# igashov/DiffLinker

Measured on AMD Instinct MI355X. Metric: molecules/sec (500-step sample_chain), higher is better.
Workload: dtype f32 (f16x3 split MFMA, fp32 accumulate)

## Files before the change

difflinker_amd/_lib.py:

```python
import ctypes
import os

import torch

_HERE = os.path.dirname(os.path.abspath(__file__))
LIB_PATH = os.environ.get('DIFFLINKER_HIP_LIB') or os.path.join(_HERE, 'libdifflinker_hip.so')
TEST_HOOKS_LIB_PATH = os.path.join(_HERE, 'libdifflinker_hip_testhooks.so')

DL_OK = 0
ABI_VERSION = 7
PRECISIONS = {'fp32': 0, 'f16x3': 1, 'f16x2': 2}
DL_ERR_TOO_MANY_ATOMS = -3


class DLConfig(ctypes.Structure):
    _fields_ = [
        ('n_dims', ctypes.c_int32), ('in_node_nf', ctypes.c_int32), ('context_node_nf', ctypes.c_int32),
        ('hidden_nf', ctypes.c_int32), ('n_layers', ctypes.c_int32), ('inv_sublayers', ctypes.c_int32),
        ('condition_time', ctypes.c_int32), ('norm_constant', ctypes.c_float),
        ('normalization_factor', ctypes.c_float), ('precision', ctypes.c_int32),
        ('attention', ctypes.c_int32), ('tanh', ctypes.c_int32), ('coords_range', ctypes.c_float),
        ('aggregation_mean', ctypes.c_int32), ('sin_embedding', ctypes.c_int32),
    ]

# ... 2 lines not shown
    _fields_ = [('in_node_nf', ctypes.c_int32), ('hidden_nf', ctypes.c_int32), ('out_node_nf', ctypes.c_int32),
                ('n_layers', ctypes.c_int32)]


class DLInpaintCoef(ctypes.Structure):
    _fields_ = [('alpha_ts', ctypes.c_float), ('c_eps', ctypes.c_float), ('sigma', ctypes.c_float),
                ('a_q', ctypes.c_float), ('b_q', ctypes.c_float), ('decode', ctypes.c_int32),
                ('inv_alpha0', ctypes.c_float), ('sigma0', ctypes.c_float), ('sigma_x', ctypes.c_float),
                ('norm_x', ctypes.c_float), ('norm_h', ctypes.c_float), ('bias_h', ctypes.c_float)]


class DLStepCoef(ctypes.Structure):
    _fields_ = [('t', ctypes.c_float), ('alpha_ts', ctypes.c_float), ('c_eps', ctypes.c_float),
                ('sigma', ctypes.c_float)]


class DLChainArgs(ctypes.Structure):
    _fields_ = [
        ('B', ctypes.c_int32), ('N', ctypes.c_int32), ('T', ctypes.c_int32), ('keep_frames', ctypes.c_int32),
        ('x', ctypes.c_void_p), ('h', ctypes.c_void_p), ('node_mask', ctypes.c_void_p),
        ('fragment_mask', ctypes.c_void_p), ('linker_mask', ctypes.c_void_p), ('edge_mask', ctypes.c_void_p),
        ('context', ctypes.c_void_p), ('noise_x', ctypes.c_void_p), ('noise_h', ctypes.c_void_p),
        ('noise_seed', ctypes.c_uint64), ('mol_offset', ctypes.c_int32), ('team', ctypes.c_int32),
        ('coefs', ctypes.c_void_p),
        ('inv_alpha0', ctypes.c_float), ('sigma0', ctypes.c_float), ('sigma_x', ctypes.c_float),
        ('norm_x', ctypes.c_float), ('norm_h', ctypes.c_float), ('bias_h', ctypes.c_float),
        ('chain', ctypes.c_void_p), ('nan_flags', ctypes.c_void_p), ('nan_step', ctypes.c_void_p),
        ('order', ctypes.c_void_p), ('workspace', ctypes.c_void_p), ('workspace_bytes', ctypes.c_size_t),
        ('mol_index', ctypes.c_void_p), ('order_first', ctypes.c_int32), ('order_count', ctypes.c_int32),
        ('q_begin', ctypes.c_void_p), ('q_end', ctypes.c_void_p), ('z_state', ctypes.c_void_p), ('skip_flags', ctypes.c_void_p),
    ]


LOSS_ROW = 8


class DLLossArgs(ctypes.Structure):
    _fields_ = [
        ('B', ctypes.c_int32), ('N', ctypes.c_int32), ('nf', ctypes.c_int32), ('T', ctypes.c_int32),
        ('timesteps', ctypes.c_int32), ('inpainting', ctypes.c_int32),
        ('xh', ctypes.c_void_p), ('node_mask', ctypes.c_void_p), ('fragment_mask', ctypes.c_void_p),
        ('linker_mask', ctypes.c_void_p), ('gamma_table', ctypes.c_void_p), ('noise_x', ctypes.c_void_p),
        ('noise_h', ctypes.c_void_p), ('noise_seed', ctypes.c_uint64), ('mol_offset', ctypes.c_int32),
        ('t_given', ctypes.c_int32), ('t_int', ctypes.c_void_p), ('t', ctypes.c_void_p), ('gamma', ctypes.c_void_p),
        ('z_t', ctypes.c_void_p), ('eps_hat', ctypes.c_void_p), ('norm_h', ctypes.c_float), ('bias_h', ctypes.c_float),
        ('prior', ctypes.c_void_p), ('rows', ctypes.c_void_p),
    ]


class DLBackwardArgs(ctypes.Structure):
    _fields_ = [
        ('B', ctypes.c_int32), ('N', ctypes.c_int32), ('in_node_nf', ctypes.c_int32), ('context_node_nf', ctypes.c_int32),
        ('condition_time', ctypes.c_int32), ('hidden_nf', ctypes.c_int32), ('n_layers', ctypes.c_int32),
        ('inv_sublayers', ctypes.c_int32), ('centering', ctypes.c_int32), ('norm_constant', ctypes.c_float),
        ('normalization_factor', ctypes.c_float), ('params', ctypes.c_void_p), ('n_params', ctypes.c_int64),
        ('xh', ctypes.c_void_p), ('t', ctypes.c_void_p), ('t_is_scalar', ctypes.c_int32), ('node_mask', ctypes.c_void_p),
        ('linker_mask', ctypes.c_void_p), ('edge_mask', ctypes.c_void_p), ('context', ctypes.c_void_p),
        ('grad_out', ctypes.c_void_p), ('grad_params', ctypes.c_void_p), ('workspace', ctypes.c_void_p),
        ('workspace_bytes', ctypes.c_size_t),
    ]


class DLSizeTrainArgs(ctypes.Structure):
    _fields_ = [
        ('B', ctypes.c_int32), ('N', ctypes.c_int32), ('in_node_nf', ctypes.c_int32), ('hidden_nf', ctypes.c_int32),
        ('out_node_nf', ctypes.c_int32), ('n_layers', ctypes.c_int32), ('batch_norm', ctypes.c_int32),
        ('params', ctypes.c_void_p), ('n_params', ctypes.c_int64), ('one_hot', ctypes.c_void_p),
        ('positions', ctypes.c_void_p), ('fragment_mask', ctypes.c_void_p), ('edge_mask', ctypes.c_void_p),
        ('logits', ctypes.c_void_p), ('batch_stats', ctypes.c_void_p), ('flags', ctypes.c_void_p),
        ('grad_logits', ctypes.c_void_p), ('grad_params', ctypes.c_void_p), ('workspace', ctypes.c_void_p),
        ('workspace_bytes', ctypes.c_size_t),
    ]


EXPORTS = ('dl_abi_version', 'dl_last_hip_error', 'dl_max_atoms', 'dl_error_string', 'dl_model_num_tensors',
           'dl_model_create', 'dl_model_destroy', 'dl_egnn_forward_fc', 'dl_sampler_step', 'dl_sample_chain_fc',
           'dl_set_profile_buffer', 'dl_profile_max_events', 'dl_pocket_workspace_bytes', 'dl_egnn_forward_pocket',
           'dl_size_model_num_tensors', 'dl_size_model_create', 'dl_size_model_destroy', 'dl_size_max_fragment_atoms',
           'dl_size_gnn_forward', 'dl_philox_fill', 'dl_egnn_forward_fc_large', 'dl_inpaint_step', 'dl_workspace_bytes',
           'dl_team_max', 'dl_egnn_forward_fc_team', 'dl_team_max_atoms',
           'dl_edm_loss_prologue', 'dl_edm_loss_epilogue', 'dl_edm_loss_grad', 'dl_egnn_backward_fc_num_params',
           'dl_egnn_backward_fc_workspace_bytes', 'dl_egnn_backward_max_atoms', 'dl_egnn_backward_fc',
           'dl_size_train_num_params', 'dl_size_train_workspace_bytes', 'dl_size_train_forward', 'dl_size_train_backward')
TEST_HOOK_EXPORTS = ('dl_debug_team_fault',)

_lib = None


class HipLibraryError(RuntimeError):
    pass


def load():
    global _lib
    if _lib is None:
        _lib = _open(LIB_PATH)
    return _lib


class test_hooks:

    def __enter__(self):
        global _lib
        self.saved = _lib
        lib = _open(TEST_HOOKS_LIB_PATH)
        lib.dl_debug_team_fault.restype = None
        lib.dl_debug_team_fault.argtypes = [ctypes.c_int32]
        _lib = lib
        return lib

    def __exit__(self, *exc):
        global _lib
        _lib.dl_debug_team_fault(0)
        _lib = self.saved
        return False

# ... 12 lines not shown
    lib.dl_last_hip_error.restype = i32
    lib.dl_max_atoms.restype = i32
    lib.dl_error_string.restype = ctypes.c_char_p
    lib.dl_error_string.argtypes = [i32]
    lib.dl_model_num_tensors.restype = i32
    lib.dl_model_num_tensors.argtypes = [ctypes.POINTER(DLConfig)]
    lib.dl_model_create.restype = i32
    lib.dl_model_create.argtypes = [ctypes.POINTER(DLConfig), ctypes.POINTER(vp), i32, ctypes.POINTER(vp)]
    lib.dl_model_destroy.restype = None
    lib.dl_model_destroy.argtypes = [vp]
    lib.dl_egnn_forward_fc.restype = i32
    lib.dl_egnn_forward_fc.argtypes = [vp, i32, i32, vp, vp, i32, vp, vp, vp, vp, vp, vp, vp, ctypes.c_size_t, vp]
    lib.dl_egnn_forward_fc_team.restype = i32
    lib.dl_egnn_forward_fc_team.argtypes = [vp, i32, i32, vp, vp, i32, vp, vp, vp, vp, vp, vp, i32, vp, ctypes.c_size_t, vp]
    lib.dl_workspace_bytes.restype = ctypes.c_size_t
    lib.dl_workspace_bytes.argtypes = [i32, i32]
    lib.dl_team_max.restype = i32
    lib.dl_team_max.argtypes = [i32]
    lib.dl_team_max_atoms.restype = i32
    lib.dl_team_max_atoms.argtypes = [i32]
    lib.dl_sampler_step.restype = i32
    lib.dl_sampler_step.argtypes = [i32, i32, i32, vp, vp, vp, vp, vp, DLStepCoef, vp, vp]
    lib.dl_set_profile_buffer.restype = None
    lib.dl_set_profile_buffer.argtypes = [vp]
    lib.dl_profile_max_events.restype = i32
    lib.dl_pocket_workspace_bytes.restype = ctypes.c_size_t
    lib.dl_pocket_workspace_bytes.argtypes = [i32, i32]
    lib.dl_egnn_forward_pocket.restype = i32
    lib.dl_egnn_forward_pocket.argtypes = [vp, i32, i32, i32, vp, vp, i32, vp, vp, vp, vp, vp, vp, ctypes.c_size_t, vp]
    lib.dl_egnn_forward_fc_large.restype = i32
    lib.dl_egnn_forward_fc_large.argtypes = [vp, i32, i32, vp, vp, i32, vp, vp, vp, vp, vp, vp, vp, ctypes.c_size_t, vp]
    lib.dl_sample_chain_fc.restype = i32
    lib.dl_sample_chain_fc.argtypes = [vp, ctypes.POINTER(DLChainArgs), vp]
    lib.dl_inpaint_step.restype = i32
    lib.dl_inpaint_step.argtypes = [i32, i32, i32] + [vp] * 10 + [DLInpaintCoef, vp, vp]
    lib.dl_philox_fill.restype = i32
    lib.dl_philox_fill.argtypes = [ctypes.c_uint64, i32, vp, i32, i32, i32, i32, i32, vp, vp, vp]
    for name in ('dl_edm_loss_prologue', 'dl_edm_loss_epilogue'):
        getattr(lib, name).restype = i32
        getattr(lib, name).argtypes = [ctypes.POINTER(DLLossArgs), vp]
    lib.dl_edm_loss_grad.restype = i32
    lib.dl_edm_loss_grad.argtypes = [ctypes.POINTER(DLLossArgs), vp, vp, vp]
    lib.dl_egnn_backward_fc_num_params.restype = ctypes.c_int64
    lib.dl_egnn_backward_fc_num_params.argtypes = [ctypes.POINTER(DLBackwardArgs)]
    lib.dl_egnn_backward_fc_workspace_bytes.restype = ctypes.c_size_t
    lib.dl_egnn_backward_fc_workspace_bytes.argtypes = [ctypes.POINTER(DLBackwardArgs)]
    lib.dl_egnn_backward_max_atoms.restype = i32
    lib.dl_egnn_backward_fc.restype = i32
    lib.dl_egnn_backward_fc.argtypes = [ctypes.POINTER(DLBackwardArgs), vp]
    lib.dl_size_train_num_params.restype = ctypes.c_int64
    lib.dl_size_train_num_params.argtypes = [ctypes.POINTER(DLSizeTrainArgs)]
    lib.dl_size_train_workspace_bytes.restype = ctypes.c_size_t
    lib.dl_size_train_workspace_bytes.argtypes = [ctypes.POINTER(DLSizeTrainArgs)]
    for name in ('dl_size_train_forward', 'dl_size_train_backward'):
        getattr(lib, name).restype = i32
        getattr(lib, name).argtypes = [ctypes.POINTER(DLSizeTrainArgs), vp]
    lib.dl_size_model_num_tensors.restype = i32
    lib.dl_size_model_num_tensors.argtypes = [ctypes.POINTER(DLSizeConfig)]
    lib.dl_size_model_create.restype = i32
    lib.dl_size_model_create.argtypes = [ctypes.POINTER(DLSizeConfig), ctypes.POINTER(vp), i32, ctypes.POINTER(vp)]
    lib.dl_size_model_destroy.restype = None
    lib.dl_size_model_destroy.argtypes = [vp]
    lib.dl_size_max_fragment_atoms.restype = i32
    lib.dl_size_gnn_forward.restype = i32
    lib.dl_size_gnn_forward.argtypes = [vp, i32, i32, vp, vp, vp, vp, vp, vp, vp, vp]
    return lib
# ... 12 lines not shown
```

difflinker_amd/csrc/egnn_fc.hip:

```cpp
#include <hip/hip_runtime.h>
#include <stdint.h>
#include <stdlib.h>
#include <string.h>
#include <math.h>
#include <cmath>

#include <algorithm>
#include <atomic>
#include <vector>

#include "../../include/difflinker_hip.h"
#include "pack_layout.h"


namespace {

constexpr int LDH = 132;
constexpr int NMAX = 55;
constexpr int NQMAX = 2 * NMAX;
constexpr int THREADS = 512;
constexpr int NWAVES = THREADS / 64;
constexpr int GWAVES = 8;
constexpr int GTHREADS = 64 * GWAVES;
constexpr int L_A = 0;
// ... 2005 lines not shown
    for (int e = tid; e < nown * D; e += THREADS) {
        const int l = e / D, d = e - l * D;
        const int pos = v.idx[rank + l * S];
        const size_t n = size_t(b) * N + pos;
        const float lm = v.lm[l], fr = v.frag[l];
        const float zt = v.z[l * DMAX + d];
        const float eh = __fmul_rn(v.A[l * DMAX + d], lm);
        float nz;
        if (philox) nz = philox_normal(seed, gmol, unsigned(pos), unsigned(q + 1), unsigned(d));
        else nz = (d < 3) ? noise_x[(q + 1) * nx_stride + n * 3 + d] : noise_h[(q + 1) * nh_stride + n * nf + d - 3];
        float zn;
        if (!decode) {
            const float mu = __fsub_rn(__fdiv_rn(zt, cf.alpha_ts), __fmul_rn(cf.c_eps, eh));
            const float zs = __fadd_rn(mu, __fmul_rn(cf.sigma, __fmul_rn(nz, lm)));
            zn = __fadd_rn(__fmul_rn(zt, fr), __fmul_rn(zs, lm));
            if (write) {
                const float o = (d < 3) ? __fmul_rn(zn, norm_x) : __fadd_rn(__fmul_rn(zn, norm_h), bias_h);
                chain_b[widx * frame + pos * D + d] = o;
            }
        } else {
            const float mu = __fmul_rn(inv_alpha0, __fsub_rn(zt, __fmul_rn(sigma0, eh)));
            const float xh = __fadd_rn(mu, __fmul_rn(sigma_x, __fmul_rn(nz, lm)));
            const float zz = __fadd_rn(__fmul_rn(zt, fr), __fmul_rn(xh, lm));
            zn = (d < 3) ? __fmul_rn(zz, norm_x) : __fadd_rn(__fmul_rn(zz, norm_h), bias_h);
        }
        v.z[l * DMAX + d] = zn;
    }
    (void)fragm;
    if (TEAM && tid == 0) v.misc[1] = 0;
    __syncthreads();
    return true;
}

template <int PREC, bool TEAM, bool ATT>
__global__ void __launch_bounds__(THREADS) sample_chain_fc_kernel(ChainArgs p) {
    __shared__ __attribute__((aligned(16))) float lds_raw[L_TOTAL];
    const Lds v = lds_view(lds_raw);
    int T, qb, qe;
    {
        const dl_chain_args& g = p.a;
        const int tid = threadIdx.x;
        int k = blockIdx.x, rank = 0, S = 1;
        const int count = g.order_count > 0 ? g.order_count : g.B;
        if constexpr (TEAM) {
            const TeamSlot ts = team_slot(blockIdx.x, g.team);
            if (ts.slot >= count) return;
            k = ts.slot; rank = ts.rank; S = g.team;
        }
        const int b = g.order ? g.order[g.order_first + k] : k;
        const int N = g.N, nf = p.md.nf, D = 3 + nf, K = g.keep_frames, B = g.B;
        const int limit = TEAM ? NQMAX : NMAX;
        T = g.T;
        qb = g.q_begin ? g.q_begin[b] : 0;
        qe = g.q_end ? g.q_end[b] : T + 1;
        if (g.skip_flags && g.skip_flags[b] != 0) return;
        const int8_t* nm = g.node_mask + size_t(b) * N;
        const size_t frame = size_t(B) * N * D;
        float* chain_b = g.chain + size_t(b) * N * D;
        const int nb = compact_atoms(v, nm, N, tid);
        if (rank == 0) {
            if (tid == 0) {
                if (TEAM) { if (nb > limit) atomicOr(&g.nan_flags[b], 4); }
                else { g.nan_flags[b] = (nb > limit) ? 4 : 0; g.nan_step[b] = -1; }
            }
            for (int kf = 0; kf < K; ++kf)
                for (int e = tid; e < N * D; e += THREADS)
                    if (nm[e / D] == 0 || nb > limit) chain_b[kf * frame + e] = 0.0f;
        }
        if (nb > limit || nb == 0) return;
        if (tid == 0) {
            if (TEAM) team_init(v, nb, S, rank, p.team_rows + size_t(k) * TEAM_MOL_BYTES, p.team_flags + size_t(k) * TEAM_MAX, p.team_fault);
            ctx_store(v, p.md, N, g.edge_mask ? g.edge_mask + size_t(b) * N * N : nullptr, p.hsave + size_t(blockIdx.x) * HS_STRIDE,
                      p.wpack, g.context ? g.context + size_t(b) * N * p.md.ctx : nullptr, 0.0f, b);
        }
        __syncthreads();
        const int nown = TEAM ? v.misc[TM_NOWN] : nb;
        if (tid < nown) {
            const size_t n = size_t(b) * N + v.idx[rank + tid * S];
            v.lm[tid] = g.linker_mask[n];
            v.frag[tid] = g.fragment_mask[n];
        }
        __syncthreads();
        build_receivers(v, nown, tid);
        const bool philox = (g.noise_x == nullptr);
        const unsigned gmol = unsigned(g.mol_offset + (g.mol_index ? g.mol_index[b] : b));
        for (int e = tid; e < nown * D; e += THREADS) {
            const int l = e / D, d = e - l * D;
            const int pos = v.idx[rank + l * S];
            const size_t n = size_t(b) * N + pos;
            float val, eps0;
            if (d < 3) { val = __fdiv_rn(g.x[n * 3 + d], g.norm_x); eps0 = philox ? 0.0f : g.noise_x[n * 3 + d]; }
            else { val = __fdiv_rn(__fsub_rn(g.h[n * nf + d - 3], g.bias_h), g.norm_h); eps0 = philox ? 0.0f : g.noise_h[n * nf + d - 3]; }
            if (philox) eps0 = philox_normal(g.noise_seed, gmol, unsigned(pos), 0u, unsigned(d));
            const float lm = v.lm[l];
            float z0 = __fadd_rn(__fmul_rn(val, v.frag[l]), __fmul_rn(__fmul_rn(eps0, lm), lm));
            if (qb > 0) z0 = g.z_state[n * D + d];
            v.z[l * DMAX + d] = z0;
        }
        __syncthreads();
    }
#pragma nounroll
    for (int q = qb; q < qe; ++q)
        if (!chain_step2<PREC, TEAM, ATT>(v, q)) return;
    if (qe <= T) {
        const auto* P = kargs<ChainArgs>();
        const int tid = lane_ids(v).tid;
        const int b = ctx_i(v, CX_MOL), nb = ctx_i(v, 0), D = 3 + P->md.nf, N = P->a.N;
        const int nown = TEAM ? ctx_i(v, TM_NOWN) : nb;
        const int S = TEAM ? ctx_i(v, TM_S) : 1, rank = TEAM ? ctx_i(v, TM_RANK) : 0;
        for (int e = tid; e < nown * D; e += THREADS) {
            const int l = e / D, d = e - l * D;
            P->a.z_state[(size_t(b) * N + v.idx[rank + l * S]) * D + d] = v.z[l * DMAX + d];
        }
        return;
    }
    {
        const auto* P = kargs<ChainArgs>();
        const int tid = lane_ids(v).tid;
        const int b = ctx_i(v, CX_MOL), nb = ctx_i(v, 0), nf = P->md.nf, D = 3 + nf;
        const int nown = TEAM ? ctx_i(v, TM_NOWN) : nb;
        const int S = TEAM ? ctx_i(v, TM_S) : 1, rank = TEAM ? ctx_i(v, TM_RANK) : 0;
        if (tid < nown) {
            const int l = tid;
            float* o = P->a.chain + size_t(b) * P->a.N * D + v.idx[rank + l * S] * D;
            o[0] = v.z[l * DMAX + 0]; o[1] = v.z[l * DMAX + 1]; o[2] = v.z[l * DMAX + 2];
            int best = 0;
            float bv = v.z[l * DMAX + 3];
            for (int kk = 1; kk < nf; ++kk) {
                const float hv = v.z[l * DMAX + 3 + kk];
                if (hv > bv) { bv = hv; best = kk; }
            }
            for (int kk = 0; kk < nf; ++kk) o[3 + kk] = (kk == best) ? 1.0f : 0.0f;
        }
        if (TEAM && tid == 0 && v.misc[TM_FAIL] != 0) atomicOr(&P->a.nan_flags[b], 8);
    }
}

__global__ void sampler_step_kernel(int total, int D, const float* __restrict__ z_t, const float* __restrict__ eps_hat,
                                    const float* __restrict__ noise, const float* __restrict__ frag,
                                    const float* __restrict__ lmask, dl_step_coef cf, float* __restrict__ z_s) {
    const int e = blockIdx.x * blockDim.x + threadIdx.x;
    if (e >= total) return;
    const int n = e / D;
    const float lm = lmask[n];
    const float zt = z_t[e];
    const float eh = __fmul_rn(eps_hat[e], lm);
    const float mu = __fsub_rn(__fdiv_rn(zt, cf.alpha_ts), __fmul_rn(cf.c_eps, eh));
    const float zs = __fadd_rn(mu, __fmul_rn(cf.sigma, __fmul_rn(noise[e], lm)));
    z_s[e] = __fadd_rn(__fmul_rn(zt, frag[n]), __fmul_rn(zs, lm));
}

thread_local int g_last_hip = 0;
#ifdef DL_TEST_HOOKS
std::atomic<int> g_team_fault{0};
#endif
unsigned long long* g_prof_buf = nullptr;

inline int take_team_fault() {
#ifdef DL_TEST_HOOKS
    int n = g_team_fault.load();
    while (n > 0 && !g_team_fault.compare_exchange_weak(n, n - 1)) {}
    return n > 0 ? 1 : 0;
#else
    return 0;
#endif
}

inline bool hip_ok(hipError_t e) {
// ... 602 lines not shown
    if (g->B < 0 || g->N < 1 || g->T < 1 || g->keep_frames < 1 || g->keep_frames > g->T || g->team < 0) return DL_ERR_BAD_ARG;
    if (g->order_first < 0 || g->order_count < 0 || g->order_first + g->order_count > g->B) return DL_ERR_BAD_ARG;
    if ((g->order_first != 0 || g->order_count != 0) && !g->order) return DL_ERR_BAD_ARG;
    if ((g->q_begin || g->q_end) && !g->z_state) return DL_ERR_BAD_ARG;
    if (m->cfg.sin_embedding) return DL_ERR_UNSUPPORTED;
    if (g->B == 0) return DL_OK;
    const int32_t count = g->order_count > 0 ? g->order_count : g->B;
    ChainArgs a;
    a.wpack = m->d_pack; a.md = dims_of(m); a.a = *g; a.prof = g_prof_buf;
    hipStream_t st = static_cast<hipStream_t>(stream);
    FcWorkspace ws;
    const int32_t rc = fc_workspace(count, g->team, g->workspace, g->workspace_bytes, st, &ws);
    if (rc != DL_OK) return rc;
    a.team_rows = ws.rows; a.team_flags = ws.flags; a.hsave = ws.hsave; a.team_fault = g->team > 1 ? take_team_fault() : 0;
    const bool f16 = m->cfg.precision != DL_PRECISION_FP32, att = m->cfg.attention != 0, two = m->cfg.precision == DL_PRECISION_F16X2 && !att;
    const void* kernel;
    if (g->team <= 1) kernel = two ? (const void*)&sample_chain_fc_kernel<2, false, false>
                             : f16 ? (att ? (const void*)&sample_chain_fc_kernel<1, false, true> : (const void*)&sample_chain_fc_kernel<1, false, false>)
                                   : (att ? (const void*)&sample_chain_fc_kernel<0, false, true> : (const void*)&sample_chain_fc_kernel<0, false, false>);
    else kernel = two ? (const void*)&sample_chain_fc_kernel<2, true, false>
                : f16 ? (att ? (const void*)&sample_chain_fc_kernel<1, true, true> : (const void*)&sample_chain_fc_kernel<1, true, false>)
                      : (att ? (const void*)&sample_chain_fc_kernel<0, true, true> : (const void*)&sample_chain_fc_kernel<0, true, false>);
    if (g->team <= 1) {
        a.a.team = 1;
        void* params[] = {&a};
        return hip_ok(hipLaunchKernel(kernel, dim3(ws.grid), dim3(THREADS), params, 0, st)) ? DL_OK : DL_ERR_HIP;
    }
    if (!hip_ok(hipMemsetAsync(g->nan_flags, 0, size_t(g->B) * sizeof(int32_t), st)) ||
        !hip_ok(hipMemsetAsync(g->nan_step, 0xFF, size_t(g->B) * sizeof(int32_t), st))) return DL_ERR_HIP;
    const hipError_t e = launch_team(kernel, ws.grid, st, &a);
    return hip_ok(e) ? DL_OK : DL_ERR_HIP;
}

namespace {
__global__ void __launch_bounds__(256) inpaint_step_kernel(int N, int nf, const float* __restrict__ z_t,
        const float* __restrict__ eps_hat, const float* __restrict__ xh_frag, const float* __restrict__ npx,
        const float* __restrict__ nph, const float* __restrict__ nqx, const float* __restrict__ nqh,
        const float* __restrict__ node_mask, const float* __restrict__ fragment_mask,
        const float* __restrict__ linker_mask, dl_inpaint_coef cf, float* __restrict__ z_s) {
    __shared__ float red[12][4];
    __shared__ float tot[12];
    const int b = blockIdx.x, tid = threadIdx.x, lane = tid & 63, wv = tid >> 6;
    const int D = 3 + nf;
    const size_t base = size_t(b) * N;
    float part[11];
#pragma unroll
    for (int k = 0; k < 11; ++k) part[k] = 0.0f;
    for (int a = tid; a < N; a += 256) {
        const float nm = node_mask[base + a];
        const float qm = cf.decode ? nm : fragment_mask[base + a];
#pragma unroll
        for (int d = 0; d < 3; ++d) {
            part[d] += npx[(base + a) * 3 + d] * nm;
            part[3 + d] += nqx[(base + a) * 3 + d] * qm;
            part[6 + d] += eps_hat[(base + a) * D + d];
        }
        part[9] += nm;
        part[10] += qm;
    }
#pragma unroll
    for (int k = 0; k < 11; ++k) {
        float s_ = part[k];
        for (int off = 32; off >= 1; off >>= 1) s_ += __shfl_xor(s_, off);
        if (lane == 0) red[k][wv] = s_;
    }
    __syncthreads();
// ... 120 lines not shown
```

difflinker_amd/edm.py:

```python
import ctypes
import functools
import os
import threading
import warnings

import numpy as np
import torch
import torch.nn.functional as F

from . import _lib, utils
from .egnn import Dynamics, DynamicsWithPockets
from .noise import PredefinedNoiseSchedule


SPLIT_CHAIN_DEFAULT = os.environ.get('DIFFLINKER_SPLIT_CHAIN', '1') == '1'


def compute_units(dev):
    return torch.cuda.get_device_properties(dev).multi_processor_count


@functools.lru_cache(maxsize=None)
def xcd_layout(bs):
    ln = -(-bs // 16)
# ... 25 lines not shown
def split_plan(sizes, linkers, n_calls, compute_units, n_layers, sublayers, min_gain=0.02, grid=48):
    B = len(sizes)
    if B > compute_units or B == 0:
        return None
    key = (tuple(sizes), tuple(linkers), n_calls, compute_units, n_layers, sublayers, min_gain, grid)
    with _CACHE_LOCK:
        if key in _PLAN_CACHE:
            return _PLAN_CACHE[key]
    table = {}
    for n, l in set(zip(sizes, linkers)):
        table[(n, l)] = (forward_cost(n, l, n_layers, sublayers, 1), forward_cost(n, l, n_layers, sublayers, 2))
    c1 = np.array([table[k][0] for k in zip(sizes, linkers)])
    c2 = np.array([table[k][1] for k in zip(sizes, linkers)])
    single = float(c1.max()) * n_calls
    lo = float(c1.min()) * n_calls
    best = None
    for i in range(1, grid):
        tau = lo + (single - lo) * i / grid
        q_end = np.clip((tau / c1).astype(np.int64), 1, n_calls)
        rest = np.nonzero(q_end < n_calls)[0]
        if rest.size == 0 or 2 * rest.size > compute_units:
            continue
        left1 = (n_calls - q_end[rest]) * c1[rest]
        teams = rest[np.lexsort((rest, -left1))]
        total = float((q_end * c1).max()) + float(((n_calls - q_end[teams]) * c2[teams]).max())
        if best is None or total < best[0]:
            best = (total, q_end.tolist(), teams.tolist())
    plan = None if best is None or best[0] > (1.0 - min_gain) * single else (best[1], best[2])
    with _CACHE_LOCK:
        if len(_PLAN_CACHE) > 64:
            _PLAN_CACHE.clear()
        _PLAN_CACHE[key] = plan
    return plan


class EDM(torch.nn.Module):
    def __init__(
            self,
            dynamics,
            in_node_nf: int,
            n_dims: int,
            timesteps: int = 1000,
            noise_schedule='learned',
            noise_precision=1e-4,
            loss_type='vlb',
            norm_values=(1., 1., 1.),
            norm_biases=(None, 0., 0.),
    ):
        super().__init__()
        if noise_schedule == 'learned':
            raise NotImplementedError("noise_schedule='learned' (GammaNetwork) is training-only and out of scope; "
                                      'released configs use polynomial_2')
        self.gamma = PredefinedNoiseSchedule(noise_schedule, timesteps=timesteps, precision=noise_precision)
        self.dynamics = dynamics
        self.in_node_nf = in_node_nf
        self.n_dims = n_dims
        self.T = timesteps
        self.norm_values = norm_values
        self.norm_biases = norm_biases
        self.noise_source = 'torch'
        self.noise_seed = 0
        self.coef_batch = None
        self.team_batch = None
        self.overflow_teams = True
        self.split_chain = SPLIT_CHAIN_DEFAULT

# ... 428 lines not shown
        xs, hs = f32(x, (bs, n, self.n_dims)), f32(h, (bs, n, nf))
        nm = node_mask.reshape(bs, n).to(torch.int8).contiguous()
        fm, lm = f32(fragment_mask, (bs, n)), f32(linker_mask, (bs, n))
        em = edge_mask.reshape(bs, n, n).to(torch.int8).contiguous() if edge_mask is not None else None
        ctx = f32(context, (bs, n, self.dynamics.context_node_nf)) if context is not None else None
        n_real = nm.ne(0).sum(1)
        order = torch.argsort(n_real, descending=True, stable=True).to(torch.int32).contiguous()
        cus = compute_units(dev)
        if 16 <= bs <= cus:
            order = order[xcd_layout(bs).to(dev)].contiguous()
        chain = torch.zeros((keep_frames, bs, n, self.n_dims + nf), device=dev)
        flags = torch.zeros(bs, dtype=torch.int32, device=dev)
        steps = torch.full((bs,), -1, dtype=torch.int32, device=dev)
        if team is None:
            team = 1 if self.dynamics._no_teams else \
                self.dynamics.team_for(bs if self.team_batch is None else max(bs, int(self.team_batch)), dev)
        over = 0
        if team == 1 and self.overflow_teams and self.team_batch is None and not self.dynamics._no_teams:
            if cus < bs <= cus + cus // 4:
                over = bs - cus
                team2 = 4 if over <= cus // 16 else 2
                while team2 > 1 and int(lib.dl_team_max(over)) < team2:
                    team2 //= 2
                if team2 < 2:
                    over = 0
            elif cus < bs < 2 * cus and not getattr(EDM, '_warned_off_sweet_spot', False):
                EDM._warned_off_sweet_spot = True
                warnings.warn(f'EDM.sample_chain: a batch of {bs} molecules on {cus} compute units runs one molecule per compute unit '
                              f'for the whole chain, so the {bs - cus} molecules beyond {cus} start only when others have finished; '
                              f'batches of k x {cus} molecules (or up to {cus + cus // 4}, whose surplus is sampled by teams beside '
                              f'the rest) use the chip evenly', RuntimeWarning, stacklevel=3)
        ws, ws_bytes = self.dynamics.workspace(bs - over, team, dev)

        plan = None
        if team == 1 and over == 0 and self.split_chain and self.team_batch is None and not self.dynamics._no_teams \
                and bs <= cus and T >= 20:
            counts = torch.stack([n_real, lm.ne(0).sum(1)]).cpu()
            sizes_h, linkers_h = counts[0].tolist(), counts[1].tolist()
            if max(sizes_h) <= int(lib.dl_max_atoms()) and min(sizes_h) > 0:
                plan = split_plan(sizes_h, linkers_h, T + 1, cus, self.dynamics.n_layers,
                                  int(getattr(self.dynamics, 'inv_sublayers', 2)))
                if plan is not None and int(lib.dl_team_max(len(plan[1]))) < 2:
                    plan = None
        q_end_t = z_state = None
        if plan is not None:
            q_end_t = torch.tensor(plan[0], dtype=torch.int32, device=dev)
            z_state = torch.empty((bs, n, self.n_dims + nf), device=dev)

        def chain_args(flags_, steps_, team_, ws_, ws_bytes_, order_, first, count, q_begin=None, q_end=None, skip=None):
            return _lib.DLChainArgs(
                q_begin=q_begin.data_ptr() if q_begin is not None else None, q_end=q_end.data_ptr() if q_end is not None else None,
                z_state=z_state.data_ptr() if z_state is not None else None, skip_flags=skip.data_ptr() if skip is not None else None,
                B=bs, N=n, T=T, keep_frames=keep_frames,
                x=xs.data_ptr(), h=hs.data_ptr(), node_mask=nm.data_ptr(), fragment_mask=fm.data_ptr(),
                linker_mask=lm.data_ptr(), edge_mask=em.data_ptr() if em is not None else None,
                context=ctx.data_ptr() if ctx is not None else None,
                noise_x=None if philox else noise_x.data_ptr(), noise_h=None if philox else noise_h.data_ptr(),
                noise_seed=seed, mol_offset=int(mol_offset), team=team_, coefs=coefs.data_ptr(),
                inv_alpha0=inv_alpha0, sigma0=sigma0, sigma_x=sigma_x,
                norm_x=float(self.norm_values[0]), norm_h=float(self.norm_values[1]), bias_h=float(self.norm_biases[1]),
                chain=chain.data_ptr(), nan_flags=flags_.data_ptr(), nan_step=steps_.data_ptr(), order=order_.data_ptr(),
                workspace=ws_.data_ptr(), workspace_bytes=ws_bytes_,
                mol_index=mol_index.data_ptr() if mol_index is not None else None, order_first=first, order_count=count)

        def side_launch(after, team_, order_, first, count, q_begin=None):
            side = self._side_stream(dev)
            flags2 = torch.empty(bs, dtype=torch.int32, device=dev)
            steps2 = torch.empty(bs, dtype=torch.int32, device=dev)
            need = int(lib.dl_workspace_bytes(count, team_))
            ws2 = self._side_workspace((dev.index, 'teams'), need, dev)
            skip = flags if q_begin is not None else None
            args2 = chain_args(flags2, steps2, team_, ws2, need, order_, first, count, q_begin=q_begin, skip=skip)
            side.wait_event(after)
            _lib.check(lib.dl_sample_chain_fc(handle, ctypes.byref(args2), ctypes.c_void_p(side.cuda_stream)),
                       'dl_sample_chain_fc (teams, beside the main launch)')
            done = torch.cuda.Event()
            done.record(side)
            cur.wait_event(done)
            for t_ in (xs, hs, nm, fm, lm, em, ctx, coefs, order_, chain, noise_x, noise_h, mol_index, q_begin, z_state, skip):
                if t_ is not None:
                    t_.record_stream(side)
            return flags | flags2, torch.where(steps2 >= 0, steps2, steps)

        args = chain_args(flags, steps, team, ws, ws_bytes, order, 0, bs - over if over else 0, q_end=q_end_t)
        profile = bool(getattr(self, 'profile_events', False))
        with torch.cuda.device(dev):
            cur = torch.cuda.current_stream(dev)
            if profile:
                ev0, ev1 = torch.cuda.Event(enable_timing=True), torch.cuda.Event(enable_timing=True)
                ev0.record(cur)
            if over:
                ready = torch.cuda.Event()
                ready.record(cur)
            _lib.check(lib.dl_sample_chain_fc(handle, ctypes.byref(args), ctypes.c_void_p(cur.cuda_stream)),
                       'dl_sample_chain_fc')
            if over:
                flags, steps = side_launch(ready, team2, order, bs - over, over)
            if plan is not None:
                after_first = torch.cuda.Event(enable_timing=profile)
                after_first.record(cur)
                self.last_split_event = after_first
                teams = sorted(plan[1], key=lambda b_: (-sizes_h[b_], b_))
                flags, steps = side_launch(after_first, 2, torch.tensor(teams, dtype=torch.int32, device=dev), 0, len(teams),
                                           q_begin=q_end_t)
            if profile:
                ev1.record(cur)
                self.last_kernel_events = (ev0, ev1)
        self._raise_on_chain_flags(flags, steps)
        bias = float(self.norm_biases[1])
        if bias != 0.0 and keep_frames > 1:
            chain[1:, :, :, self.n_dims:] += bias * (1.0 - node_mask.to(chain.dtype).reshape(bs, n, 1))
        return chain

    def philox_noise_bank(self, n_samples, n_nodes, device, mol_offset=0, seed=None, n_draws=None):
        if torch.device(device).type != 'cuda':
            raise RuntimeError('the Philox noise bank is generated on the GPU (no CPU fallback)')
        if seed is None:
            seed = int(self.noise_seed)
            self.noise_seed = seed + 1
        n_draws = self.T + 2 if n_draws is None else int(n_draws)
        noise_x = torch.empty((n_draws, n_samples, n_nodes, self.n_dims), device=device)
        noise_h = torch.empty((n_draws, n_samples, n_nodes, self.in_node_nf), device=device)
        with torch.cuda.device(device):
            stream = torch.cuda.current_stream(device).cuda_stream
            _lib.check(_lib.load().dl_philox_fill(int(seed) & 0xFFFFFFFFFFFFFFFF, int(mol_offset), None, n_samples, n_nodes,
                                                  self.in_node_nf, 0, n_draws, noise_x.data_ptr(), noise_h.data_ptr(),
                                                  ctypes.c_void_p(stream)), 'dl_philox_fill')
        return noise_x, noise_h
# ... 269 lines not shown
```

include/difflinker_hip.h:

```cpp
#ifndef DIFFLINKER_HIP_H
#define DIFFLINKER_HIP_H

#include <stddef.h>
#include <stdint.h>

#ifdef __cplusplus
extern "C" {
#endif

#define DL_ABI_VERSION 7

typedef enum dl_status {
    DL_OK = 0,
    DL_ERR_BAD_ARG = -1,
    DL_ERR_UNSUPPORTED = -2,
    DL_ERR_TOO_MANY_ATOMS = -3,
    DL_ERR_HIP = -4,
    DL_ERR_NO_DEVICE = -5,
    DL_ERR_ALLOC = -6
} dl_status;

typedef enum dl_precision { DL_PRECISION_FP32 = 0, DL_PRECISION_F16X3 = 1, DL_PRECISION_F16X2 = 2 } dl_precision;

typedef struct dl_config {
// ... 56 lines not shown

typedef struct dl_chain_args {
    int32_t B, N, T, keep_frames;
    const float* x;
    const float* h;
    const int8_t* node_mask;
    const float* fragment_mask;
    const float* linker_mask;
    const int8_t* edge_mask;
    const float* context;
    const float* noise_x;
    const float* noise_h;
    uint64_t noise_seed;
    int32_t mol_offset;
    int32_t team;
    const dl_step_coef* coefs;
    float inv_alpha0, sigma0, sigma_x;
    float norm_x, norm_h, bias_h;
    float* chain;
    int32_t* nan_flags;
    int32_t* nan_step;
    const int32_t* order;
    void* workspace;
    size_t workspace_bytes;
    const int32_t* mol_index;
    int32_t order_first, order_count;
    const int32_t* q_begin;
    const int32_t* q_end;
    float* z_state;
    const int32_t* skip_flags;
} dl_chain_args;

int32_t dl_sample_chain_fc(const dl_model* m, const dl_chain_args* args, void* stream);

int32_t dl_team_max(int32_t B);
int32_t dl_team_max_atoms(int32_t team);
#ifdef DL_TEST_HOOKS
void dl_debug_team_fault(int32_t launches);
#endif
int32_t dl_egnn_forward_fc_team(const dl_model* m, int32_t B, int32_t N, const float* xh, const float* t,
                                int32_t t_is_scalar, const int8_t* node_mask, const float* linker_mask,
                                const int8_t* edge_mask, const float* context, float* out, int32_t* nan_flags,
                                int32_t team, void* workspace, size_t workspace_bytes, void* stream);

typedef struct dl_inpaint_coef {
    float alpha_ts, c_eps, sigma;
    float a_q, b_q;
    int32_t decode;
    float inv_alpha0, sigma0, sigma_x;
    float norm_x, norm_h, bias_h;
} dl_inpaint_coef;
int32_t dl_inpaint_step(int32_t B, int32_t N, int32_t nf, const float* z_t, const float* eps_hat, const float* xh_frag,
                        const float* noise_px, const float* noise_ph, const float* noise_qx, const float* noise_qh,
                        const float* node_mask, const float* fragment_mask, const float* linker_mask,
                        dl_inpaint_coef coef, float* z_s, void* stream);

int32_t dl_philox_fill(uint64_t seed, int32_t mol_offset, const int32_t* mol_index, int32_t B, int32_t N, int32_t nf, int32_t draw0,
                       int32_t n_draws, float* noise_x, float* noise_h, void* stream);

#define DL_LOSS_ROW 8
typedef struct dl_loss_args {
    int32_t B, N, nf;
    int32_t T;
    int32_t timesteps;
    int32_t inpainting;
    const float* xh;
// ... 103 lines not shown
```

Measured before the change: 542.8.

## Add single-launch join kernel where finished small molecules help large ones

Adds a join variant of the sampling chain kernel. Each molecule runs alone on its own block; after a small helper molecule finishes, its block meets a large owner molecule through a global-memory handshake. The pair then finishes the owner's remaining diffusion steps as a 2-block team. This replaces the split-plan path, which needed separate launches, and aims to balance the tail of per-molecule work across CUs. In exchange it relies on co-resident blocks spinning on global flags, with a timeout that poisons the pair.

New measurement: 588.0, median of 6. 1.08x the previous value.

```diff
diff --git a/difflinker_amd/_lib.py b/difflinker_amd/_lib.py
--- a/difflinker_amd/_lib.py
+++ b/difflinker_amd/_lib.py
@@ -58,6 +58,13 @@
     ]
 
 
+class DLJoinArgs(ctypes.Structure):
+    _fields_ = [
+        ('teams', ctypes.c_int32), ('team_of', ctypes.c_void_p), ('team_mol', ctypes.c_void_p),
+        ('workspace', ctypes.c_void_p), ('workspace_bytes', ctypes.c_size_t), ('wait_ticks', ctypes.c_void_p),
+    ]
+
+
 LOSS_ROW = 8
 
 
@@ -107,7 +114,8 @@
            'dl_team_max', 'dl_egnn_forward_fc_team', 'dl_team_max_atoms',
            'dl_edm_loss_prologue', 'dl_edm_loss_epilogue', 'dl_edm_loss_grad', 'dl_egnn_backward_fc_num_params',
            'dl_egnn_backward_fc_workspace_bytes', 'dl_egnn_backward_max_atoms', 'dl_egnn_backward_fc',
-           'dl_size_train_num_params', 'dl_size_train_workspace_bytes', 'dl_size_train_forward', 'dl_size_train_backward')
+           'dl_size_train_num_params', 'dl_size_train_workspace_bytes', 'dl_size_train_forward', 'dl_size_train_backward',
+           'dl_join_workspace_bytes', 'dl_sample_chain_fc_join')
 TEST_HOOK_EXPORTS = ('dl_debug_team_fault',)
 
 _lib = None
@@ -186,6 +194,10 @@
     lib.dl_egnn_forward_fc_large.argtypes = [vp, i32, i32, vp, vp, i32, vp, vp, vp, vp, vp, vp, vp, ctypes.c_size_t, vp]
     lib.dl_sample_chain_fc.restype = i32
     lib.dl_sample_chain_fc.argtypes = [vp, ctypes.POINTER(DLChainArgs), vp]
+    lib.dl_join_workspace_bytes.restype = ctypes.c_size_t
+    lib.dl_join_workspace_bytes.argtypes = [i32]
+    lib.dl_sample_chain_fc_join.restype = i32
+    lib.dl_sample_chain_fc_join.argtypes = [vp, ctypes.POINTER(DLChainArgs), ctypes.POINTER(DLJoinArgs), vp]
     lib.dl_inpaint_step.restype = i32
     lib.dl_inpaint_step.argtypes = [i32, i32, i32] + [vp] * 10 + [DLInpaintCoef, vp, vp]
     lib.dl_philox_fill.restype = i32
diff --git a/difflinker_amd/csrc/egnn_fc.hip b/difflinker_amd/csrc/egnn_fc.hip
--- a/difflinker_amd/csrc/egnn_fc.hip
+++ b/difflinker_amd/csrc/egnn_fc.hip
@@ -2061,76 +2061,63 @@
     return true;
 }
 
-template <int PREC, bool TEAM, bool ATT>
-__global__ void __launch_bounds__(THREADS) sample_chain_fc_kernel(ChainArgs p) {
-    __shared__ __attribute__((aligned(16))) float lds_raw[L_TOTAL];
-    const Lds v = lds_view(lds_raw);
-    int T, qb, qe;
-    {
-        const dl_chain_args& g = p.a;
-        const int tid = threadIdx.x;
-        int k = blockIdx.x, rank = 0, S = 1;
-        const int count = g.order_count > 0 ? g.order_count : g.B;
-        if constexpr (TEAM) {
-            const TeamSlot ts = team_slot(blockIdx.x, g.team);
-            if (ts.slot >= count) return;
-            k = ts.slot; rank = ts.rank; S = g.team;
-        }
-        const int b = g.order ? g.order[g.order_first + k] : k;
-        const int N = g.N, nf = p.md.nf, D = 3 + nf, K = g.keep_frames, B = g.B;
-        const int limit = TEAM ? NQMAX : NMAX;
-        T = g.T;
-        qb = g.q_begin ? g.q_begin[b] : 0;
-        qe = g.q_end ? g.q_end[b] : T + 1;
-        if (g.skip_flags && g.skip_flags[b] != 0) return;
-        const int8_t* nm = g.node_mask + size_t(b) * N;
-        const size_t frame = size_t(B) * N * D;
-        float* chain_b = g.chain + size_t(b) * N * D;
-        const int nb = compact_atoms(v, nm, N, tid);
-        if (rank == 0) {
-            if (tid == 0) {
-                if (TEAM) { if (nb > limit) atomicOr(&g.nan_flags[b], 4); }
-                else { g.nan_flags[b] = (nb > limit) ? 4 : 0; g.nan_step[b] = -1; }
-            }
-            for (int kf = 0; kf < K; ++kf)
-                for (int e = tid; e < N * D; e += THREADS)
-                    if (nm[e / D] == 0 || nb > limit) chain_b[kf * frame + e] = 0.0f;
-        }
-        if (nb > limit || nb == 0) return;
+template <bool TEAM>
+__device__ __forceinline__ bool chain_begin(const ChainArgs& p, const Lds& v, int b, int rank, int S, int qb, char* rows,
+                                            unsigned* flags) {
+    const dl_chain_args& g = p.a;
+    const int tid = threadIdx.x;
+    const int N = g.N, nf = p.md.nf, D = 3 + nf, K = g.keep_frames, B = g.B;
+    const int limit = TEAM ? NQMAX : NMAX;
+    if (g.skip_flags && g.skip_flags[b] != 0) return false;
+    const int8_t* nm = g.node_mask + size_t(b) * N;
+    const size_t frame = size_t(B) * N * D;
+    float* chain_b = g.chain + size_t(b) * N * D;
+    const int nb = compact_atoms(v, nm, N, tid);
+    if (rank == 0) {
         if (tid == 0) {
-            if (TEAM) team_init(v, nb, S, rank, p.team_rows + size_t(k) * TEAM_MOL_BYTES, p.team_flags + size_t(k) * TEAM_MAX, p.team_fault);
-            ctx_store(v, p.md, N, g.edge_mask ? g.edge_mask + size_t(b) * N * N : nullptr, p.hsave + size_t(blockIdx.x) * HS_STRIDE,
-                      p.wpack, g.context ? g.context + size_t(b) * N * p.md.ctx : nullptr, 0.0f, b);
-        }
-        __syncthreads();
-        const int nown = TEAM ? v.misc[TM_NOWN] : nb;
-        if (tid < nown) {
-            const size_t n = size_t(b) * N + v.idx[rank + tid * S];
-            v.lm[tid] = g.linker_mask[n];
-            v.frag[tid] = g.fragment_mask[n];
-        }
-        __syncthreads();
-        build_receivers(v, nown, tid);
-        const bool philox = (g.noise_x == nullptr);
-        const unsigned gmol = unsigned(g.mol_offset + (g.mol_index ? g.mol_index[b] : b));
-        for (int e = tid; e < nown * D; e += THREADS) {
-            const int l = e / D, d = e - l * D;
-            const int pos = v.idx[rank + l * S];
-            const size_t n = size_t(b) * N + pos;
-            float val, eps0;
-            if (d < 3) { val = __fdiv_rn(g.x[n * 3 + d], g.norm_x); eps0 = philox ? 0.0f : g.noise_x[n * 3 + d]; }
-            else { val = __fdiv_rn(__fsub_rn(g.h[n * nf + d - 3], g.bias_h), g.norm_h); eps0 = philox ? 0.0f : g.noise_h[n * nf + d - 3]; }
-            if (philox) eps0 = philox_normal(g.noise_seed, gmol, unsigned(pos), 0u, unsigned(d));
-            const float lm = v.lm[l];
-            float z0 = __fadd_rn(__fmul_rn(val, v.frag[l]), __fmul_rn(__fmul_rn(eps0, lm), lm));
-            if (qb > 0) z0 = g.z_state[n * D + d];
-            v.z[l * DMAX + d] = z0;
-        }
-        __syncthreads();
-    }
-#pragma nounroll
-    for (int q = qb; q < qe; ++q)
-        if (!chain_step2<PREC, TEAM, ATT>(v, q)) return;
+            if (TEAM) { if (nb > limit) atomicOr(&g.nan_flags[b], 4); }
+            else { g.nan_flags[b] = (nb > limit) ? 4 : 0; g.nan_step[b] = -1; }
+        }
+        for (int kf = 0; kf < K; ++kf)
+            for (int e = tid; e < N * D; e += THREADS)
+                if (nm[e / D] == 0 || nb > limit) chain_b[kf * frame + e] = 0.0f;
+    }
+    if (nb > limit || nb == 0) return false;
+    if (tid == 0) {
+        if (TEAM) team_init(v, nb, S, rank, rows, flags, p.team_fault);
+        ctx_store(v, p.md, N, g.edge_mask ? g.edge_mask + size_t(b) * N * N : nullptr, p.hsave + size_t(blockIdx.x) * HS_STRIDE,
+                  p.wpack, g.context ? g.context + size_t(b) * N * p.md.ctx : nullptr, 0.0f, b);
+    }
+    __syncthreads();
+    const int nown = TEAM ? v.misc[TM_NOWN] : nb;
+    if (tid < nown) {
+        const size_t n = size_t(b) * N + v.idx[rank + tid * S];
+        v.lm[tid] = g.linker_mask[n];
+        v.frag[tid] = g.fragment_mask[n];
+    }
+    __syncthreads();
+    build_receivers(v, nown, tid);
+    const bool philox = (g.noise_x == nullptr);
+    const unsigned gmol = unsigned(g.mol_offset + (g.mol_index ? g.mol_index[b] : b));
+    for (int e = tid; e < nown * D; e += THREADS) {
+        const int l = e / D, d = e - l * D;
+        const int pos = v.idx[rank + l * S];
+        const size_t n = size_t(b) * N + pos;
+        float val, eps0;
+        if (d < 3) { val = __fdiv_rn(g.x[n * 3 + d], g.norm_x); eps0 = philox ? 0.0f : g.noise_x[n * 3 + d]; }
+        else { val = __fdiv_rn(__fsub_rn(g.h[n * nf + d - 3], g.bias_h), g.norm_h); eps0 = philox ? 0.0f : g.noise_h[n * nf + d - 3]; }
+        if (philox) eps0 = philox_normal(g.noise_seed, gmol, unsigned(pos), 0u, unsigned(d));
+        const float lm = v.lm[l];
+        float z0 = __fadd_rn(__fmul_rn(val, v.frag[l]), __fmul_rn(__fmul_rn(eps0, lm), lm));
+        if (qb > 0) z0 = g.z_state[n * D + d];
+        v.z[l * DMAX + d] = z0;
+    }
+    __syncthreads();
+    return true;
+}
+
+template <bool TEAM>
+__device__ __forceinline__ void chain_end(const Lds& v, int qe, int T) {
     if (qe <= T) {
         const auto* P = kargs<ChainArgs>();
         const int tid = lane_ids(v).tid;
@@ -2163,6 +2150,109 @@
         }
         if (TEAM && tid == 0 && v.misc[TM_FAIL] != 0) atomicOr(&P->a.nan_flags[b], 8);
     }
+}
+
+template <int PREC, bool TEAM, bool ATT>
+__global__ void __launch_bounds__(THREADS) sample_chain_fc_kernel(ChainArgs p) {
+    __shared__ __attribute__((aligned(16))) float lds_raw[L_TOTAL];
+    const Lds v = lds_view(lds_raw);
+    int T, qb, qe;
+    {
+        const dl_chain_args& g = p.a;
+        int k = blockIdx.x, rank = 0, S = 1;
+        const int count = g.order_count > 0 ? g.order_count : g.B;
+        if constexpr (TEAM) {
+            const TeamSlot ts = team_slot(blockIdx.x, g.team);
+            if (ts.slot >= count) return;
+            k = ts.slot; rank = ts.rank; S = g.team;
+        }
+        const int b = g.order ? g.order[g.order_first + k] : k;
+        T = g.T;
+        qb = g.q_begin ? g.q_begin[b] : 0;
+        qe = g.q_end ? g.q_end[b] : T + 1;
+        if (!chain_begin<TEAM>(p, v, b, rank, S, qb, TEAM ? p.team_rows + size_t(k) * TEAM_MOL_BYTES : nullptr,
+                               TEAM ? p.team_flags + size_t(k) * TEAM_MAX : nullptr)) return;
+    }
+#pragma nounroll
+    for (int q = qb; q < qe; ++q)
+        if (!chain_step2<PREC, TEAM, ATT>(v, q)) return;
+    chain_end<TEAM>(v, qe, T);
+}
+
+constexpr unsigned JW_READY = 1u, JW_DEAD = 2u, JW_HERE = 3u, JW_POISON = 0xFFFFFFFFu;
+constexpr unsigned long long JOIN_WAIT_TICKS = 100000000ull * 20;
+constexpr int JOIN_WORDS = 4;
+
+struct JoinArgs {
+    ChainArgs c;
+    const int32_t* team_of;
+    const int32_t* team_mol;
+    unsigned* words;
+    unsigned long long* wait_ticks;
+};
+
+__device__ __forceinline__ unsigned join_meet(const Lds& v, unsigned* words, int rank, unsigned mine, unsigned long long* wait) {
+    asm volatile("s_waitcnt vmcnt(0)" ::: "memory");
+    __syncthreads();
+    if (threadIdx.x == 0) {
+        typedef __attribute__((address_space(1))) unsigned gu32;
+        gu32* w = reinterpret_cast<gu32*>(reinterpret_cast<unsigned long long>(words));
+        __builtin_amdgcn_fence(__ATOMIC_RELEASE, "agent");
+        __hip_atomic_store(w + rank, mine, __ATOMIC_RELAXED, __HIP_MEMORY_SCOPE_AGENT);
+        const unsigned long long t0 = __builtin_amdgcn_s_memrealtime();
+        unsigned other = 0;
+        if (mine != JW_DEAD && mine != JW_POISON) {
+            for (;;) {
+                other = __hip_atomic_load(w + (1 - rank), __ATOMIC_RELAXED, __HIP_MEMORY_SCOPE_AGENT);
+                if (other != 0) break;
+                if (__builtin_amdgcn_s_memrealtime() - t0 > JOIN_WAIT_TICKS) {
+                    __hip_atomic_store(w + rank, JW_POISON, __ATOMIC_RELAXED, __HIP_MEMORY_SCOPE_AGENT);
+                    other = JW_POISON;
+                    break;
+                }
+                __builtin_amdgcn_s_sleep(32);
+            }
+            __builtin_amdgcn_fence(__ATOMIC_ACQUIRE, "agent");
+        }
+        if (wait) wait[rank] = __builtin_amdgcn_s_memrealtime() - t0;
+        v.misc[TM_FAIL] = int(other);
+    }
+    __syncthreads();
+    return unsigned(v.misc[TM_FAIL]);
+}
+
+template <int PREC, bool ATT>
+__global__ void __launch_bounds__(THREADS) sample_chain_fc_kernel_join(JoinArgs p) {
+    __shared__ __attribute__((aligned(16))) float lds_raw[L_TOTAL];
+    const Lds v = lds_view(lds_raw);
+    const int k = blockIdx.x;
+    const int b = p.c.a.order ? p.c.a.order[k] : k;
+    const int T = p.c.a.T, qe = p.c.a.q_end[b];
+    bool alive = chain_begin<false>(p.c, v, b, 0, 1, 0, nullptr, nullptr);
+    if (alive) {
+#pragma nounroll
+        for (int q = 0; q < qe; ++q)
+            if (!chain_step2<PREC, false, ATT>(v, q)) { alive = false; break; }
+    }
+    if (alive) chain_end<false>(v, qe, T);
+    const int j = p.team_of[b];
+    if (j < 0) return;
+    const int rank = qe <= T ? 0 : 1;
+    const int bo = rank == 0 ? b : p.team_mol[j];
+    const unsigned mine = rank == 1 ? JW_HERE : alive ? JW_READY : JW_DEAD;
+    const unsigned other = join_meet(v, p.words + size_t(j) * JOIN_WORDS, rank, mine,
+                                     p.wait_ticks ? p.wait_ticks + size_t(j) * 2 : nullptr);
+    if (mine == JW_DEAD || other == JW_DEAD) return;
+    if (other == JW_POISON) {
+        if (threadIdx.x == 0) atomicOr(&p.c.a.nan_flags[bo], 8);
+        return;
+    }
+    const int qb = p.c.a.q_end[bo];
+    if (!chain_begin<true>(p.c, v, bo, rank, 2, qb, p.c.team_rows + size_t(j) * TEAM_MOL_BYTES,
+                           p.c.team_flags + size_t(j) * TEAM_MAX)) return;
+#pragma nounroll
+    for (int q = qb; q <= T; ++q) chain_step2<PREC, true, ATT>(v, q);
+    chain_end<true>(v, T + 1, T);
 }
 
 __global__ void sampler_step_kernel(int total, int D, const float* __restrict__ z_t, const float* __restrict__ eps_hat,
@@ -2831,6 +2921,48 @@
     return hip_ok(e) ? DL_OK : DL_ERR_HIP;
 }
 
+size_t dl_join_workspace_bytes(int32_t teams) {
+    if (teams <= 0) return 0;
+    return size_t(teams) * (TEAM_MOL_BYTES + TEAM_MAX * sizeof(unsigned) + JOIN_WORDS * sizeof(unsigned));
+}
+
+int32_t dl_sample_chain_fc_join(const dl_model* m, const dl_chain_args* g, const dl_join_args* jn, void* stream) {
+    if (!m || !g || !jn) return DL_ERR_BAD_ARG;
+    if (!g->x || !g->h || !g->node_mask || !g->fragment_mask || !g->linker_mask ||
+        !g->coefs || !g->chain || !g->nan_flags || !g->nan_step) return DL_ERR_BAD_ARG;
+    if ((g->noise_x == nullptr) != (g->noise_h == nullptr)) return DL_ERR_BAD_ARG;
+    if (m->cfg.context_node_nf > 0 && !g->context) return DL_ERR_BAD_ARG;
+    if (g->B < 1 || g->N < 1 || g->T < 1 || g->keep_frames < 1 || g->keep_frames > g->T || g->team > 1 || g->team < 0) return DL_ERR_BAD_ARG;
+    if (g->order_first != 0 || g->order_count != 0 || g->q_begin || g->skip_flags || !g->q_end || !g->z_state) return DL_ERR_BAD_ARG;
+    if (jn->teams < 1 || 2 * jn->teams > g->B || !jn->team_of || !jn->team_mol) return DL_ERR_BAD_ARG;
+    if (!jn->workspace || jn->workspace_bytes < dl_join_workspace_bytes(jn->teams) ||
+        (reinterpret_cast<uintptr_t>(jn->workspace) & 15u) != 0) return DL_ERR_BAD_ARG;
+    if (m->cfg.sin_embedding) return DL_ERR_UNSUPPORTED;
+    int dev = 0, cus = 0;
+    if (!hip_ok(hipGetDevice(&dev)) || !hip_ok(hipDeviceGetAttribute(&cus, hipDeviceAttributeMultiprocessorCount, dev))) return DL_ERR_HIP;
+    if (g->B > cus) return DL_ERR_BAD_ARG;
+    JoinArgs a;
+    a.c.wpack = m->d_pack; a.c.md = dims_of(m); a.c.a = *g; a.c.a.team = 1; a.c.prof = g_prof_buf;
+    hipStream_t st = static_cast<hipStream_t>(stream);
+    FcWorkspace ws;
+    const int32_t rc = fc_workspace(g->B, 1, g->workspace, g->workspace_bytes, st, &ws);
+    if (rc != DL_OK) return rc;
+    char* w = static_cast<char*>(jn->workspace);
+    a.c.hsave = ws.hsave;
+    a.c.team_rows = w;
+    a.c.team_flags = reinterpret_cast<unsigned*>(w + size_t(jn->teams) * TEAM_MOL_BYTES);
+    a.words = a.c.team_flags + size_t(jn->teams) * TEAM_MAX;
+    a.c.team_fault = take_team_fault();
+    a.team_of = jn->team_of; a.team_mol = jn->team_mol;
+    a.wait_ticks = reinterpret_cast<unsigned long long*>(jn->wait_ticks);
+    if (!hip_ok(hipMemsetAsync(a.c.team_flags, 0, size_t(jn->teams) * (TEAM_MAX + JOIN_WORDS) * sizeof(unsigned), st))) return DL_ERR_HIP;
+    const bool f16 = m->cfg.precision != DL_PRECISION_FP32, att = m->cfg.attention != 0, two = m->cfg.precision == DL_PRECISION_F16X2 && !att;
+    const void* kernel = two ? (const void*)&sample_chain_fc_kernel_join<2, false>
+                       : f16 ? (att ? (const void*)&sample_chain_fc_kernel_join<1, true> : (const void*)&sample_chain_fc_kernel_join<1, false>)
+                             : (att ? (const void*)&sample_chain_fc_kernel_join<0, true> : (const void*)&sample_chain_fc_kernel_join<0, false>);
+    return hip_ok(launch_team(kernel, g->B, st, &a)) ? DL_OK : DL_ERR_HIP;
+}
+
 namespace {
 __global__ void __launch_bounds__(256) inpaint_step_kernel(int N, int nf, const float* __restrict__ z_t,
         const float* __restrict__ eps_hat, const float* __restrict__ xh_frag, const float* __restrict__ npx,
diff --git a/difflinker_amd/edm.py b/difflinker_amd/edm.py
--- a/difflinker_amd/edm.py
+++ b/difflinker_amd/edm.py
@@ -81,6 +81,45 @@
             _PLAN_CACHE.clear()
         _PLAN_CACHE[key] = plan
     return plan
+
+
+def join_plan(sizes, linkers, n_calls, compute_units, n_layers, sublayers, margin=0.03):
+    split = split_plan(sizes, linkers, n_calls, compute_units, n_layers, sublayers)
+    if split is None:
+        return None
+    key = ('join', tuple(sizes), tuple(linkers), n_calls, compute_units, n_layers, sublayers, margin)
+    with _CACHE_LOCK:
+        if key in _PLAN_CACHE:
+            return _PLAN_CACHE[key]
+    owners = list(split[1])
+    in_team = set(owners)
+    rest = [b for b in range(len(sizes)) if b not in in_team]
+    plan = None
+    if len(rest) >= len(owners):
+        c1 = [forward_cost(n, l, n_layers, sublayers, 1) for n, l in zip(sizes, linkers)]
+        owners.sort(key=lambda b: (-c1[b], b))
+        rest.sort(key=lambda b: (c1[b], b))
+        helpers = rest[:len(owners)]
+        q_end = [n_calls] * len(sizes)
+        for o, hp in zip(owners, helpers):
+            arrive = n_calls * c1[hp] * (1.0 + margin)
+            q_end[o] = int(min(max(-(-arrive // c1[o]), 1), n_calls - 1))
+        plan = (q_end, owners, helpers)
+    with _CACHE_LOCK:
+        if len(_PLAN_CACHE) > 64:
+            _PLAN_CACHE.clear()
+        _PLAN_CACHE[key] = plan
+    return plan
+
+
+def join_makespan(plan, sizes, linkers, n_calls, n_layers, sublayers):
+    q_end, owners, helpers = plan
+    c1 = [forward_cost(n, l, n_layers, sublayers, 1) for n, l in zip(sizes, linkers)]
+    end = [n_calls * c for c in c1]
+    for o, hp in zip(owners, helpers):
+        start = max(q_end[o] * c1[o], end[hp])
+        end[o] = start + (n_calls - q_end[o]) * forward_cost(sizes[o], linkers[o], n_layers, sublayers, 2)
+    return max(end)
 
 
 class EDM(torch.nn.Module):
@@ -575,19 +614,23 @@
                               f'the rest) use the chip evenly', RuntimeWarning, stacklevel=3)
         ws, ws_bytes = self.dynamics.workspace(bs - over, team, dev)
 
-        plan = None
+        plan = join = None
         if team == 1 and over == 0 and self.split_chain and self.team_batch is None and not self.dynamics._no_teams \
                 and bs <= cus and T >= 20:
             counts = torch.stack([n_real, lm.ne(0).sum(1)]).cpu()
             sizes_h, linkers_h = counts[0].tolist(), counts[1].tolist()
             if max(sizes_h) <= int(lib.dl_max_atoms()) and min(sizes_h) > 0:
-                plan = split_plan(sizes_h, linkers_h, T + 1, cus, self.dynamics.n_layers,
-                                  int(getattr(self.dynamics, 'inv_sublayers', 2)))
+                sub = int(getattr(self.dynamics, 'inv_sublayers', 2))
+                plan = split_plan(sizes_h, linkers_h, T + 1, cus, self.dynamics.n_layers, sub)
                 if plan is not None and int(lib.dl_team_max(len(plan[1]))) < 2:
                     plan = None
+                if plan is not None:
+                    join = join_plan(sizes_h, linkers_h, T + 1, cus, self.dynamics.n_layers, sub)
+                    if join is not None:
+                        plan = None
         q_end_t = z_state = None
-        if plan is not None:
-            q_end_t = torch.tensor(plan[0], dtype=torch.int32, device=dev)
+        if plan is not None or join is not None:
+            q_end_t = torch.tensor((join or plan)[0], dtype=torch.int32, device=dev)
             z_state = torch.empty((bs, n, self.n_dims + nf), device=dev)
 
         def chain_args(flags_, steps_, team_, ws_, ws_bytes_, order_, first, count, q_begin=None, q_end=None, skip=None):
@@ -635,8 +678,22 @@
             if over:
                 ready = torch.cuda.Event()
                 ready.record(cur)
-            _lib.check(lib.dl_sample_chain_fc(handle, ctypes.byref(args), ctypes.c_void_p(cur.cuda_stream)),
-                       'dl_sample_chain_fc')
+            if join is not None:
+                _, owners, helpers = join
+                team_of = [-1] * bs
+                for j_, (o_, hp_) in enumerate(zip(owners, helpers)):
+                    team_of[o_] = team_of[hp_] = j_
+                maps = torch.tensor(team_of + owners, dtype=torch.int32, device=dev)
+                need = int(lib.dl_join_workspace_bytes(len(owners)))
+                jws = self._side_workspace((dev.index, 'join'), need, dev)
+                jargs = _lib.DLJoinArgs(teams=len(owners), team_of=maps.data_ptr(), team_mol=maps.data_ptr() + 4 * bs,
+                                        workspace=jws.data_ptr(), workspace_bytes=need, wait_ticks=None)
+                _lib.check(lib.dl_sample_chain_fc_join(handle, ctypes.byref(args), ctypes.byref(jargs),
+                                                       ctypes.c_void_p(cur.cuda_stream)), 'dl_sample_chain_fc_join')
+                self.last_split_event = None
+            else:
+                _lib.check(lib.dl_sample_chain_fc(handle, ctypes.byref(args), ctypes.c_void_p(cur.cuda_stream)),
+                           'dl_sample_chain_fc')
             if over:
                 flags, steps = side_launch(ready, team2, order, bs - over, over)
             if plan is not None:
diff --git a/include/difflinker_hip.h b/include/difflinker_hip.h
--- a/include/difflinker_hip.h
+++ b/include/difflinker_hip.h
@@ -112,6 +112,18 @@
 } dl_chain_args;
 
 int32_t dl_sample_chain_fc(const dl_model* m, const dl_chain_args* args, void* stream);
+
+typedef struct dl_join_args {
+    int32_t teams;
+    const int32_t* team_of;
+    const int32_t* team_mol;
+    void* workspace;
+    size_t workspace_bytes;
+    uint64_t* wait_ticks;
+} dl_join_args;
+
+size_t dl_join_workspace_bytes(int32_t teams);
+int32_t dl_sample_chain_fc_join(const dl_model* m, const dl_chain_args* args, const dl_join_args* join, void* stream);
 
 int32_t dl_team_max(int32_t B);
 int32_t dl_team_max_atoms(int32_t team);
```
